# mryndzionek/composable-sdr

Measured on AMD Instinct MI355X. Metric: MS/s CF32 throughput, 256-ch PFB+FM pipeline, higher is better.
Workload: dtype f32; 1 GPU; cfg3: 256-ch firpfbch(m=7,As=80)+dcBlocker+freqdem(kf=0.3) on synthetic CF32, AGC off (-a 0), 262144 frames/step (512 MiB in, 256 MiB out), HBM-resident; channels=256, demod=fm, mix=False, route=fused-256|k_tile256<FM>, preheat_steps=12154, collective=none, rccl_ranks=1

## Files before the change

### composable_sdr_amd/csrc/fused_common.h

```cpp
#pragma once
#include "fused.h"
#include "run_split.h"

#include <cmath>
#include <cstdlib>
#include <vector>

namespace csdr {
namespace {

constexpr int M256 = 256;
constexpr int P = 14;
constexpr int NB = 16;
constexpr int FS_X = 272;
constexpr int FS_Z = 289;
constexpr int RS_Z = 18;
constexpr int RS_Y = 17;
constexpr int LDS_F2 = 16 * FS_Z;
constexpr int E_OFF = 4096;
constexpr int LOOKBACK = 10;
constexpr unsigned SPIN_LIMIT = 1u << 24;

typedef unsigned long long u64;
typedef float v2f __attribute__((ext_vector_type(2)));
// ... 310 lines not shown
{
    float2 s = T[tid & 15];
    float2 t;
    t = dpp2<0x111>(s); s = cfma(t, A.b256[1], s);
    t = dpp2<0x112>(s); s = cfma(t, A.b256[2], s);
    t = dpp2<0x114>(s); s = cfma(t, A.b256[4], s);
    t = dpp2<0x118>(s); s = cfma(t, A.b256[8], s);
    const int f = (tid >> 4) & 15;
    const int srcl = (tid & 48) | ((f - 1) & 15);
    float2 r = make_float2(__shfl(s.x, srcl), __shfl(s.y, srcl));
    return f ? r : make_float2(0.f, 0.f);
}


constexpr int WU = 6;


struct RunArgs {
    TileArgs t;
    RunSplit split;
    PhaseK pk;
    uint32_t nruns;
    float l2beta;
    uint32_t prio_div;
    uint32_t trace_light;
    const float4 *prev_tail;
    uint32_t indep;
    uint32_t pair_align;
    uint32_t wu_batch6;
    uint32_t wu, wu_rot;
    uint32_t tile_step;
    uint32_t nowu;
    float2 *cpre, *side;
};
constexpr int DCFIX_F = 113;

__device__ __forceinline__ float2 wg_sum(float2 v, float2 *red, int tid)
{
#pragma unroll
    for (int d = 32; d >= 1; d >>= 1) { v.x += __shfl_xor(v.x, d); v.y += __shfl_xor(v.y, d); }
    if ((tid & 63) == 0) red[tid >> 6] = v;
    __syncthreads();
    const float2 r = cadd(cadd(red[0], red[1]), cadd(red[2], red[3]));
    __syncthreads();
    return r;
}

__device__ __forceinline__ void row_scan4(float &x0, float &x1, float &x2, float &x3, float &s0, float &s1, float &s2, float &s3,
                                          float b1, float b2, float b4, float b8, float na)
{
    asm volatile(
        "v_mov_b32_e32 %4, %0\n\t"
        "v_mov_b32_e32 %5, %1\n\t"
        "v_mov_b32_e32 %6, %2\n\t"
        "v_mov_b32_e32 %7, %3\n\t"
        "v_fmac_f32_dpp %4, %4, %8 row_shr:1 row_mask:0xf bank_mask:0xf\n\t"
        "v_fmac_f32_dpp %5, %5, %8 row_shr:1 row_mask:0xf bank_mask:0xf\n\t"
        "v_fmac_f32_dpp %6, %6, %8 row_shr:1 row_mask:0xf bank_mask:0xf\n\t"
        "v_fmac_f32_dpp %7, %7, %8 row_shr:1 row_mask:0xf bank_mask:0xf\n\t"
        "v_fmac_f32_dpp %4, %4, %9 row_shr:2 row_mask:0xf bank_mask:0xf\n\t"
        "v_fmac_f32_dpp %5, %5, %9 row_shr:2 row_mask:0xf bank_mask:0xf\n\t"
        "v_fmac_f32_dpp %6, %6, %9 row_shr:2 row_mask:0xf bank_mask:0xf\n\t"
        "v_fmac_f32_dpp %7, %7, %9 row_shr:2 row_mask:0xf bank_mask:0xf\n\t"
        "v_fmac_f32_dpp %4, %4, %10 row_shr:4 row_mask:0xf bank_mask:0xf\n\t"
        "v_fmac_f32_dpp %5, %5, %10 row_shr:4 row_mask:0xf bank_mask:0xf\n\t"
        "v_fmac_f32_dpp %6, %6, %10 row_shr:4 row_mask:0xf bank_mask:0xf\n\t"
        "v_fmac_f32_dpp %7, %7, %10 row_shr:4 row_mask:0xf bank_mask:0xf\n\t"
        "v_fmac_f32_dpp %4, %4, %11 row_shr:8 row_mask:0xf bank_mask:0xf\n\t"
// ... 62 lines not shown
```

### composable_sdr_amd/csrc/fused_v2_common.h

```cpp
#pragma once
#include "fused_common.h"

namespace csdr {
namespace {

typedef float v4f __attribute__((ext_vector_type(4)));
#ifndef V2_DMA_AUX
#define V2_DMA_AUX ""
#endif
#ifndef V2_DMA_AUX_STREAM
#define V2_DMA_AUX_STREAM V2_DMA_AUX
#endif

__device__ __forceinline__ void bar()
{
    asm volatile("s_waitcnt lgkmcnt(0)\n\ts_barrier" ::: "memory");
}
__device__ __forceinline__ float opaque_v(float x) { asm volatile("" : "+v"(x)); return x; }

__device__ __forceinline__ unsigned dma_offset(int tid)
{
    const int wave = tid >> 6, lane = tid & 63;
    const int slot = 64 * wave + lane, q = slot >> 3, i = (slot & 7) ^ ((q >> 1) & 7);
    return (unsigned)(8 * q + i) * 16u;
// ... 97 lines not shown
#pragma unroll
    for (int i = 5; i >= 0; i--) {
        pA = __builtin_elementwise_fma(pA, zA, (v2f){k.c[i], k.c[i]});
        pB = __builtin_elementwise_fma(pB, zB, (v2f){k.c[i], k.c[i]});
    }
    const v2f tA = pA * sA, tB = pB * sB;
    const v2f hpv = {k.hp, k.hp}, piv = {k.pi, k.pi};
    const v2f thA = hpv - tA, thB = hpv - tB;
    const v2f uA = {sel_abs_gt(q[0].y, q[0].x, thA.x, tA.x), sel_abs_gt(q[1].y, q[1].x, thA.y, tA.y)};
    const v2f uB = {sel_abs_gt(q[2].y, q[2].x, thB.x, tB.x), sel_abs_gt(q[3].y, q[3].x, thB.y, tB.y)};
    const v2f wA = piv - uA, wB = piv - uB;
    m[0] = copysignf(sel_neg(q[0].x, wA.x, uA.x), q[0].y);
    m[1] = copysignf(sel_neg(q[1].x, wA.y, uA.y), q[1].y);
    m[2] = copysignf(sel_neg(q[2].x, wB.x, uB.x), q[2].y);
    m[3] = copysignf(sel_neg(q[3].x, wB.y, uB.y), q[3].y);
}

template <int CTRL> __device__ __forceinline__ float dpp_keep(float old, float v)
{
    return __int_as_float(__builtin_amdgcn_update_dpp(__float_as_int(old), __float_as_int(v), CTRL, 0xf, 0xf, false));
}

}
template <size_t OFF> __device__ __forceinline__ unsigned kernarg_u32_s()
{
    unsigned v = 0;
#if defined(__HIP_DEVICE_COMPILE__)
    typedef __attribute__((address_space(4))) const char *kptr;
    kptr ka = (kptr)__builtin_amdgcn_kernarg_segment_ptr();
    asm volatile("s_load_dword %0, %1, %2\n\ts_waitcnt lgkmcnt(0)" : "=s"(v) : "s"(ka), "n"(OFF) : "memory");
#endif
    return v;
}
template <size_t OFF> __device__ __forceinline__ float2 *kernarg_ptr_s()
{
    float2 *p = nullptr;
#if defined(__HIP_DEVICE_COMPILE__)
    typedef __attribute__((address_space(4))) const char *kptr;
    kptr ka = (kptr)__builtin_amdgcn_kernarg_segment_ptr();
    unsigned long long v;
    asm volatile("s_load_dwordx2 %0, %1, %2\n\ts_waitcnt lgkmcnt(0)" : "=s"(v) : "s"(ka), "n"(OFF) : "memory");
    p = reinterpret_cast<float2 *>(v);
#endif
    return p;
}

}
```

### composable_sdr_amd/csrc/kernels_fused.hip

```cpp
#include "fused_common.h"
#include <cstring>

namespace csdr {

namespace {

#define STAMP(i) do { if (A.trace && tid == 0) A.trace[(size_t)b * 16 + (i)] = __builtin_amdgcn_s_memtime(); } while (0)

template <bool FM>
__global__ __launch_bounds__(256) void k_tile256(TileArgs A)
{
    __shared__ __attribute__((aligned(16))) float2 R[LDS_F2];
    __shared__ float2 tw_s[M256];
    __shared__ float2 Tt[2][16];
    __shared__ float2 carry_s[2];
    __shared__ unsigned tile_s;

    const int tid = threadIdx.x;
    if (tid == 0) tile_s = atomicAdd(A.ticket, 1u);
    tw_s[tid] = A.tw[tid];
    __syncthreads();
    const unsigned b = tile_s;
    if (b >= A.nb) return;
    STAMP(0);
// ... 232 lines not shown
            for (int f = 0; f < NB; f++) if (f < nvalid) o[f] = v[f];
        }
    }
    STAMP(11);
}


}


__global__ __launch_bounds__(256) void k_save_tail(const float4 *__restrict__ src, float4 *__restrict__ dst)
{
    const unsigned i = blockIdx.x * 256u + threadIdx.x;
    dst[i] = src[i];
}

__global__ __launch_bounds__(64) void k_shard_gather(const float *__restrict__ src, float *__restrict__ dst, uint32_t c0, uint32_t G, uint32_t rem,
                                                     uint32_t nf, uint32_t t0, uint32_t w)
{
    const uint32_t m = blockIdx.x;
    for (uint32_t i = threadIdx.x; i < rem * w; i += 64) dst[((size_t)m * nf + t0) * w + i] = src[(size_t)(c0 + G * m) * rem * w + i];
}

struct FusedPlan : ChainPlan {
    using ChainPlan::ChainPlan;
    std::string kernel;
    uint32_t max_nb = 0, epoch = 0;
    float *d_taps = nullptr;
    float2 *d_tw = nullptr, *d_wpre = nullptr;
    float2 *d_yhist[2] = {nullptr, nullptr}, *d_vend[2] = {nullptr, nullptr}, *d_rp[2] = {nullptr, nullptr};
    unsigned *d_ticket = nullptr, *d_yflag = nullptr, *d_status = nullptr;
    u64 *d_agg = nullptr, *d_ylast = nullptr;
    float2 *d_cpre = nullptr, *d_side = nullptr, *d_rt = nullptr;
    bool nowu = false;
    u64 *d_trace = nullptr;
    uint32_t run_min_tiles = 1024;
    float slot_weight[8] = {1.f, 1.f, 1.f, 1.f, 1.f, 1.f, 1.f, 1.f};
    uint32_t slot_pairs[8] = {0, 0, 0, 0, 0, 0, 0, 0};
    bool have_pairs = false;
    uint32_t resident_wgs_v2 = 512;
    bool use_v3 = false;
    float *d_shard_tail = nullptr;
    float4 *d_tail[3] = {nullptr, nullptr, nullptr};
    int tail_w = 0;
    bool tail_valid = false, save_tails = false;
    TileArgs proto;

    int init();
    const char *name() const override { return kernel.c_str(); }
    bool tile_major_ok(uint32_t nf) const override;
    void keep_tail() override { save_tails = cfg.G == 1; }
    bool can_overlap(uint32_t nf) const override;
    bool tail_recorded() const override { return save_tails && tail_valid; }
    int status(unsigned *st) override;
    int trace(unsigned long long *out, uint32_t ntiles) override;
    int reset_state(hipStream_t s) override;
    int run(const FusedCall &call, void *out, hipStream_t s, KernelTimer *timer) override;
    bool v2_call(uint32_t nf) const { return cfg.G == 1 && cfg.c0 == 0 && cfg.C == cfg.M && nf / NB >= run_min_tiles; }
};

int ChainPlan::process(const FusedCall &call, hipStream_t s, KernelTimer *timer)
{
    if (!call.nf) return 0;
    if ((call.tile_major && !tile_major_ok(call.nf)) || (call.indep && !can_overlap(call.nf))) {
        set_error("fused: internal: tile-major output or an independent launch requested from a call that cannot run as one");
        return -1;
    }
// ... 60 lines not shown
    kernel = cfg.fm ? "k_tile256<FM>" : "k_tile256<CF32>";
    max_nb = (cfg.max_nf + NB - 1) / NB;
    if ((r = mem.alloc(&d_taps, sizeof(float) * cfg.M * cfg.p))) return r;
    if ((r = mem.alloc(&d_tw, sizeof(float2) * cfg.M))) return r;
    if ((r = mem.alloc(&d_wpre, sizeof(float2) * 2 * cfg.M))) return r;
    for (int i = 0; i < 2; i++) {
        if ((r = mem.alloc(&d_yhist[i], sizeof(float2) * 13 * cfg.M))) return r;
        if ((r = mem.alloc(&d_vend[i], sizeof(float2)))) return r;
        if ((r = mem.alloc(&d_rp[i], sizeof(float2) * (cfg.G > 1 ? cfg.M : cfg.C)))) return r;
    }
    if (cfg.G > 1 && (r = mem.alloc(&d_shard_tail, sizeof(float2) * cfg.M * NB))) return r;
    for (int i = 0; i < 3; i++) {
        if ((r = mem.alloc(&d_tail[i], sizeof(float4) * 2048 * (WU + 1)))) return r;
        CSDR_HIP(hipMemset(d_tail[i], 0, sizeof(float4) * 2048 * (WU + 1)));
    }
    tail_valid = true;
    if ((r = mem.alloc(&d_ticket, sizeof(unsigned)))) return r;
    if ((r = mem.alloc(&d_status, sizeof(unsigned)))) return r;
    if ((r = mem.alloc(&d_yflag, sizeof(unsigned) * max_nb))) return r;
    if ((r = mem.alloc(&d_agg, sizeof(u64) * 2 * max_nb))) return r;
    if ((r = mem.alloc(&d_ylast, sizeof(u64) * (size_t)cfg.M * max_nb))) return r;
    if (const char *e = diag_env("CSDR_RUN_MIN_TILES")) run_min_tiles = (uint32_t)atol(e);
    if (cfg.mix && (r = mem.alloc(&d_premix, (size_t)cfg.C * cfg.max_nf * (cfg.fm ? 4 : 8)))) return r;
    if (diag_env("CSDR_TRACE")) {
        if ((r = mem.alloc(&d_trace, sizeof(u64) * 16 * max_nb))) return r;
        CSDR_HIP(hipMemset(d_trace, 0, sizeof(u64) * 16 * max_nb));
    }
    nowu = cfg.G == 1 && cfg.c0 == 0 && cfg.C == cfg.M && cfg.dc_block && dc_window_ok(cfg.dc, (DCFIX_F - 1) * 256.0) &&
           !(diag_env("CSDR_NOWU") && atoi(diag_env("CSDR_NOWU")) == 0);
    if (nowu) {
        if ((r = mem.alloc(&d_cpre, sizeof(float2) * 2050))) return r;
        if ((r = mem.alloc(&d_side, sizeof(float2) * 2048 * 4 * DCFIX_F))) return r;
        if ((r = mem.alloc(&d_rt, sizeof(float2) * 2 * DCFIX_F * 4))) return r;
        CSDR_HIP(hipMemset(d_cpre, 0, sizeof(float2) * 2050));
    }
    CSDR_HIP(hipMemcpy(d_taps, cfg.taps, sizeof(float) * cfg.M * cfg.p, hipMemcpyHostToDevice));
    std::vector<float2> tw(cfg.M);
    for (uint32_t k1 = 0; k1 < 16; k1++)
        for (uint32_t b1 = 0; b1 < 16; b1++) {
            const double a = -2.0 * 3.14159265358979323846 * (double)(b1 * k1) / (double)cfg.M;
            tw[16 * k1 + b1] = make_float2((float)std::cos(a), (float)std::sin(a));
        }
    const std::vector<float2> wpre = premix_table();
    CSDR_HIP(hipMemcpy(d_tw, tw.data(), sizeof(float2) * cfg.M, hipMemcpyHostToDevice));
    CSDR_HIP(hipMemcpy(d_wpre, wpre.data(), sizeof(float2) * 2 * cfg.M, hipMemcpyHostToDevice));
    if (nowu) {
        std::vector<float2> rt((size_t)2 * DCFIX_F * 4);
        dc_state_response(cfg, wpre.data(), 15u, (uint32_t)DCFIX_F, 126u, rt.data());
        CSDR_HIP(hipMemcpy(d_rt, rt.data(), sizeof(float2) * rt.size(), hipMemcpyHostToDevice));
    }
    CSDR_HIP(hipMemset(d_status, 0, sizeof(unsigned)));
    CSDR_HIP(hipMemset(d_yflag, 0, sizeof(unsigned) * max_nb));
    CSDR_HIP(hipMemset(d_agg, 0, sizeof(u64) * 2 * max_nb));

    TileArgs &A = proto;
    A = TileArgs{};
    A.taps = d_taps; A.tw = d_tw; A.wpre = d_wpre;
    A.ticket = d_ticket; A.agg = d_agg; A.ylast = d_ylast; A.yflag = d_yflag; A.status = d_status;
    A.c0 = cfg.c0; A.C = cfg.C; A.fm_ref = cfg.fm_ref; A.trace = d_trace;
    const double beta = cfg.dc_block ? (double)cfg.dc.beta : 0.0;
    A.alpha = cfg.dc_block ? (float)(1.0 - beta) : 0.0f;
    A.beta = (float)beta;
    for (int k = 0; k < LOOKBACK + 2; k++) A.wtile[k] = (float)std::pow(beta, 4096.0 * k);
    for (int k = 0; k < 16; k++) A.b16[k] = (float)std::pow(beta, 16.0 * k);
    for (int k = 0; k < 17; k++) A.b256[k] = (float)std::pow(beta, 256.0 * k);
    for (int k = 0; k < 16; k++) A.bj[k] = (float)std::pow(beta, (double)k);
    if (const char *e = diag_env("CSDR_CUS")) { if (atoi(e) > 0 && (uint32_t)atoi(e) < cus) cus = (uint32_t)atoi(e); }
    resident_wgs_v2 = (uint32_t)(cus * run256_v2_blocks_per_cu(cfg.fm, cfg.G));
    if (const char *e = diag_env("CSDR_RESIDENT_WGS")) resident_wgs_v2 = (uint32_t)atol(e);
#ifdef CSDR_WITH_RUN256_V3
    if (const char *e = diag_env("CSDR_RUN_V3")) use_v3 = atoi(e) != 0;
#endif
    if (const char *e = diag_env("CSDR_RUN_WEIGHTS")) {
        int k = 0;
        for (const char *q = e; *q && k < 8; k++) { slot_weight[k] = (float)atof(q); q = strchr(q, ','); if (!q) break; q++; }
    }
    if (const char *e = diag_env("CSDR_RUN_PAIRS")) {
        int k = 0;
        for (const char *q = e; *q && k < 8; k++) { slot_pairs[k] = (uint32_t)atol(q); q = strchr(q, ','); if (!q) break; q++; }
        have_pairs = true;
    }
    return 0;
}

int FusedPlan::reset_state(hipStream_t s)
{
    for (int i = 0; i < 2; i++) {
        CSDR_HIP(hipMemsetAsync(d_yhist[i], 0, sizeof(float2) * 13 * cfg.M, s));
        CSDR_HIP(hipMemsetAsync(d_vend[i], 0, sizeof(float2), s));
        CSDR_HIP(hipMemsetAsync(d_rp[i], 0, sizeof(float2) * (cfg.G > 1 ? cfg.M : cfg.C), s));
    }
    CSDR_HIP(hipMemsetAsync(d_tail[0], 0, sizeof(float4) * 2048 * (WU + 1), s));
    tail_w = 0; tail_valid = true;
    return 0;
}

bool FusedPlan::tile_major_ok(uint32_t nf) const
{
    if (cfg.fm || cfg.mix || nf % NB || !nf) return false;
    if (cfg.G > 1) return (uint64_t)cfg.C * nf * 8u < (1ull << 32);
    return cfg.c0 == 0 && cfg.C == cfg.M && nf / NB >= run_min_tiles;
}

bool FusedPlan::can_overlap(uint32_t nf) const
{
    return save_tails && tail_valid && v2_call(nf) && nf % NB == 0 && !cfg.mix;
}

int FusedPlan::run(const FusedCall &call, void *out, hipStream_t s, KernelTimer *timer)
{
    const FusedConfig &c = cfg;
    const uint32_t nf = call.nf;
    int r;
    TileArgs A = proto;
    A.x = call.d_in;
    A.out = out;
    A.yhist_in = d_yhist[cur]; A.yhist_out = d_yhist[cur ^ 1];
    A.vend_in = d_vend[cur];   A.vend_out = d_vend[cur ^ 1];
    A.rp_in = d_rp[cur];       A.rp_out = d_rp[cur ^ 1];
    A.out_stride = nf; A.out_t0 = 0;
    if (call.tile_major) A.out_stride = NB;
    A.parity0 = (uint32_t)(frames_done & 1);
    const uint32_t nb_full = nf / NB;
    const bool shard = c.G > 1;
    if (shard && (uint64_t)c.C * nf * (c.fm ? 4u : 8u) >= (1ull << 32)) { set_error("fused: interleaved shard output of %u frames exceeds 4 GiB", nf); return -1; }
// ... 1 lines not shown
    if ((nb_full >= run_min_tiles && whole_band) || shard) {
        const bool v2 = true;
        const bool v3 = !shard && use_v3;
        kernel = v3 ? (c.fm ? "k_run256v3<FM>" : "k_run256v3<CF32>") : (c.fm ? "k_run256v2<FM>" : "k_run256v2<CF32>");
        if (shard) kernel += "/G" + std::to_string(c.G);
        RunArgs RA{};
        A.nf = nb_full * NB; A.nb = nb_full;
        RA.t = A; RA.pk = phase_consts(c.fm_ref);
        uint32_t nruns = v3 ? cus : resident_wgs_v2;
        if (v3) { if (const char *e = diag_env("CSDR_V3_RUNS")) nruns = (uint32_t)atol(e); }
        if (nruns > A.nb / 8) nruns = A.nb / 8;
        if (nruns < 1) nruns = 1;
        RA.nruns = nruns;
        static const float v2_weight_cf[8] = {1.2f, 0.8f, 1.f, 1.f, 1.f, 1.f, 1.f, 1.f};
        static const float v2_weight_fm[8] = {1.24f, 0.76f, 1.f, 1.f, 1.f, 1.f, 1.f, 1.f};
        static const float v2_weight_fm3[8] = {1.6f, 1.f, 0.6f, 1.f, 1.f, 1.f, 1.f, 1.f};
        const float *v2_weight = c.fm ? ((cus && nruns == 3 * cus) ? v2_weight_fm3 : v2_weight_fm) : v2_weight_cf;
        static const float equal_weight[8] = {1.f, 1.f, 1.f, 1.f, 1.f, 1.f, 1.f, 1.f};
        static const bool pd_equal = diag_env("CSDR_PD_EQUAL") != nullptr;
        RA.split = make_split(A.nb, nruns, cus, (call.indep && pd_equal) ? equal_weight : ((v2 && !diag_env("CSDR_RUN_WEIGHTS")) ? v2_weight : slot_weight),
                              have_pairs ? slot_pairs : nullptr);
        { const char *e = diag_env("CSDR_PRIO_ROT"); RA.prio_div = e ? (atoi(e) ? cus : 0u) : (v2 ? 0u : cus); }
        { const char *e = diag_env("CSDR_TRACE"); RA.trace_light = (e && atoi(e) == 2) ? 1u : 0u; }
        { const char *e = diag_env("CSDR_WU"); RA.wu = e ? (uint32_t)atoi(e) : (uint32_t)WU; }
        { const char *e = diag_env("CSDR_WU_ROT"); RA.wu_rot = e ? (uint32_t)atoi(e) : 0u; }
        RA.pair_align = (v2 && (c.fm || diag_env("CSDR_PAIR_ALIGN_CF"))) ? 1u : 0u;
        { const char *e = diag_env("CSDR_WU_BATCH6"); RA.wu_batch6 = e ? (uint32_t)atoi(e) : 1u; }
        RA.l2beta = c.dc_block ? (float)std::log2((double)c.dc.beta) : -1000.0f;
        RA.tile_step = call.tile_major ? c.C * 128u : (uint32_t)NB * (c.fm ? 4u : 8u);
        const bool whole = nf == nb_full * NB;
        RA.indep = call.indep ? 1u : 0u;
        RA.nowu = (nowu && !shard && !v3 && !RA.indep && nruns >= 2 && nruns <= 2048) ? 1u : 0u;
        RA.cpre = d_cpre; RA.side = d_side;
        RA.prev_tail = d_tail[tail_w];
        if (save_tails && !shard && v2 && whole && nb_full >= WU + 1) {
            const int nxt = (tail_w + 1) % 3;
            static const bool nocopy = diag_env("CSDR_PD_NOCOPY") != nullptr;
            if (!nocopy) hipLaunchKernelGGL(k_save_tail, dim3(2048 * (WU + 1) / 256), dim3(256), 0, s,
                                            reinterpret_cast<const float4 *>(call.d_in + (size_t)(nb_full - (WU + 1)) * 4096), d_tail[nxt]);
            if (call.ev_tail) CSDR_HIP(hipEventRecord(call.ev_tail, s));
            tail_w = nxt; tail_valid = true;
        } else tail_valid = false;
        if (timer && (r = timer->begin(s))) return r;
        if (nb_full == 0) {  }
#ifdef CSDR_WITH_RUN256_V3
        else if (v3) { if ((r = run256_v3_launch(&RA, c.fm, nruns, s))) return r; }
#endif
        else if ((r = run256_v2_launch(&RA, c.fm, c.G, nruns, s))) return r;
        if (RA.nowu && nb_full && (r = run256_dcfix_launch(&RA, c.fm, nruns, d_rt, s))) return r;
        if (timer && (r = timer->end(s))) return r;
        const uint32_t rem = nf - nb_full * NB;
        if (rem) {
            if (nb_full) cur ^= 1;
            TileArgs T = proto;
            T.x = call.d_in + (size_t)nb_full * NB * c.M; T.out = A.out;
            if (shard) { T.c0 = 0; T.C = c.M; T.out = d_shard_tail; }
            T.yhist_in = d_yhist[cur]; T.yhist_out = d_yhist[cur ^ 1];
            T.vend_in = d_vend[cur];   T.vend_out = d_vend[cur ^ 1];
            T.rp_in = d_rp[cur];       T.rp_out = d_rp[cur ^ 1];
            if (++epoch == 0) epoch = 1;
            T.epoch = epoch; T.nf = rem; T.nb = 1; T.out_stride = nf; T.out_t0 = nb_full * NB;
            if (shard) { T.out_stride = rem; T.out_t0 = 0; }
            T.parity0 = (uint32_t)((frames_done + nb_full * NB) & 1);
            CSDR_HIP(hipMemsetAsync(d_ticket, 0, sizeof(unsigned), s));
            if (c.fm) hipLaunchKernelGGL(k_tile256<true>, dim3(1), dim3(256), 0, s, T);
            else hipLaunchKernelGGL(k_tile256<false>, dim3(1), dim3(256), 0, s, T);
            if (shard) hipLaunchKernelGGL(k_shard_gather, dim3(c.C), dim3(64), 0, s, (const float *)d_shard_tail, (float *)A.out, c.c0, c.G, rem,
                                          nf, nb_full * NB, c.fm ? 1u : 2u);
        }
    } else {
        kernel = c.fm ? "k_tile256<FM>" : "k_tile256<CF32>";
        tail_valid = false;
        if (++epoch == 0) epoch = 1;
        A.epoch = epoch; A.nf = nf; A.nb = (nf + NB - 1) / NB;
        CSDR_HIP(hipMemsetAsync(d_ticket, 0, sizeof(unsigned), s));
        if (timer && (r = timer->begin(s))) return r;
        if (c.fm) hipLaunchKernelGGL(k_tile256<true>, dim3(A.nb), dim3(256), 0, s, A);
        else hipLaunchKernelGGL(k_tile256<false>, dim3(A.nb), dim3(256), 0, s, A);
        if (timer && (r = timer->end(s))) return r;
    }
    CSDR_HIP(hipGetLastError());
    return 0;
// ... 20 lines not shown
```

### composable_sdr_amd/csrc/kernels_fused_v2.hip

```cpp
#ifndef V2_FM_PACKED
#define V2_FM_PACKED 1
#endif
#ifndef V2_ABLATE
#define V2_ABLATE 0
#endif

#ifndef V2_COLSCAN
#define V2_COLSCAN 0
#endif
#ifndef V2_PAIR
#define V2_PAIR 1
#endif
#ifndef V2_STORE_AUX
#define V2_STORE_AUX ""
#endif
#ifndef V2_PAIR_CF
#define V2_PAIR_CF 0
#endif
#ifndef V2_BAR_E
#define V2_BAR_E 0
#endif
#ifndef V2_PAD
#define V2_PAD 1
#endif
#ifndef V2_ONE_WGS
#define V2_ONE_WGS 3
#endif
#ifndef V2_ONE_BURST
#define V2_ONE_BURST 1
#endif
#ifndef V2_SNOP
#define V2_SNOP ""
#endif

#include "fused_v2_common.h"
#include <cstddef>
#include <type_traits>

namespace csdr {
namespace {

constexpr unsigned V2_FSB = 2048u + (V2_PAD ? 128u : 0u);
constexpr int V2_FS2 = (int)V2_FSB / 8;
constexpr int V2_BUF = 16 * V2_FS2;
constexpr int V2_STASH = 2 * V2_BUF;
constexpr int V2_AUX2 = 256 + 32 + 256 + (V2_COLSCAN ? 512 : 0);
constexpr int V2_F2 = V2_STASH + V2_AUX2;
constexpr int V2_F2_ONE = V2_BUF + V2_AUX2 + P * M256 / 2;
#define V2_ZSW(f) (V2_PAD ? (((f) >> 1) & 7) : ((f) & 7))
#ifndef V2_RSWN
#define V2_RSWN V2_PAD
#endif
#define V2_RSW(a) (V2_RSWN ? ((a) & 7) : (((a) >> 1) & 7))

struct V2Args {
    RunArgs r;
};

template <bool FM, int G>
__global__ __launch_bounds__(256, (FM && G == 1) ? V2_ONE_WGS : 2) void k_run256v2(V2Args VA)
{
    static_assert(G == 1 || G == 2 || G == 4 || G == 8, "interleaved shards: G = 2, 4, 8");
    constexpr int NK1 = 16 / G;
    constexpr bool ONE = FM && G == 1;
    const RunArgs &RA = VA.r;
    const TileArgs &A = RA.t;
    __shared__ __attribute__((aligned(16))) float2 L[(ONE && V2_ONE_WGS >= 3) ? V2_F2_ONE : V2_F2];
    float2 *R = L, *ST = L + (ONE ? V2_BUF : V2_STASH), *Tt = ST + 256, *red = Tt + 16;
    float2 *tw_s = red + 16;
    float2 *TRc = tw_s + 256, *Ec = TRc + 256;
    (void)TRc; (void)Ec;
    float *TP = reinterpret_cast<float *>(L + (ONE ? V2_BUF : V2_STASH) + V2_AUX2);
    float2 *H = ONE ? L : L + V2_BUF;
    float2 *HS = ONE ? reinterpret_cast<float2 *>(TP) : H;
    float2 *E = ST;
    const int tid = threadIdx.x, j = tid;
    const unsigned w = blockIdx.x;
    unsigned first, last;
    run_range(RA.split, w, first, last);
    if (RA.pair_align) {
        first &= ~1u;
        if (last != A.nb) last &= ~1u;
    }
    const float4 *x4 = reinterpret_cast<const float4 *>(A.x);
    const int col_off = 16 * (j >> 4) + 2 * (((j & 15) >> 1) ^ V2_RSW(j >> 4)) + (j & 1);
    const unsigned goff = V2_RSWN ? dma_offset_rsw(tid) : dma_offset(tid);
    const unsigned wave_u = (unsigned)__builtin_amdgcn_readfirstlane(tid >> 6);
    const unsigned lds_wave = (unsigned)(size_t)(__attribute__((address_space(3))) float2 *)R + V2_FSB * (wave_u >> 1) + 1024u * (wave_u & 1u);

#ifndef V2_TRACE
// ... 121 lines not shown
    const int st_i = XIDX(tid >> 4), st_j1 = ((tid & 15) - (int)(G > 1 ? A.c0 : 0u)) / G;
    const bool st_own = G == 1 || ((((tid & 15) - (int)A.c0) & (G - 1)) == 0 && (tid & 15) >= (int)A.c0);
    const int st_idx = G == 1 ? (tid & 15) * 16 + st_i : (st_own ? ((st_i / NK1) * NK1 + st_j1) * 16 + st_i : 0);
    if (st_own) ST[st_idx] = (FM && !cold) ? A.rp_in[tid] : make_float2(0.f, 0.f);
    __syncthreads();
    if (FM && cold) {
        w2 = cmul(w2, Wa);
        v2f acc = {0.f, 0.f};
#pragma unroll
        for (int n = P - 1; n >= 0; n--) {
            const float2 s2 = (n == P - 1) ? w2 : wa[NB - 1 - n];
            acc = __builtin_elementwise_fma((v2f){s2.x, s2.y}, (v2f){h[n], h[n]}, acc);
        }
        HS[j] = to_f2(acc);
        __syncthreads();
        v2f vv[16];
        if (tid < 16) {
#pragma unroll
            for (int a = 0; a < 16; a++) vv[a] = to_v(HS[16 * a + tid]);
            fft16_v(vv);
#pragma unroll
            for (int i = (G > 1 ? 0 : 1); i < 16; i++) vv[i] = cmul_v(vv[i], to_v(tw_s[16 * ((XIDX(i) + (G > 1 ? (int)A.c0 : 0)) & 15) + tid]));
#pragma unroll
            for (int i = 0; i < 16; i++) HS[256 + 16 * XIDX(i) + tid] = to_f2(vv[i]);
        }
        __syncthreads();
        if (tid < 16) {
#pragma unroll
            for (int b = 0; b < 16; b++) vv[b] = to_v(HS[256 + 16 * (G * (tid % NK1)) + b]);
            fft16_v(vv);
#pragma unroll
            for (int i = 0; i < 16; i++) ST[tid * 16 + i] = to_f2(vv[i]);
            if (G == 1 && RA.nowu) {
                if (tid >= 14) RA.side[((size_t)w * 4 + (tid - 14)) * DCFIX_F] = to_f2(vv[13]);
                else if (tid <= 1) RA.side[((size_t)w * 4 + 2 + tid) * DCFIX_F] = to_f2(vv[2]);
            }
        }
        __syncthreads();
    }

    if (ONE) {
#pragma unroll
        for (int n = 0; n < P; n++) TP[M256 * n + j] = h[n];
    }
    const v2f Wav = to_v(Wa), Wbv = to_v(Wb);
    const float na = opaque_v(-A.alpha), be = opaque_v(A.beta);
    const float kJ = -A.alpha * exp2f((float)j * RA.l2beta);
    const float b256 = A.b256[1];
    const FmK2 fk = {{opaque_v(9.999993443e-01f), opaque_v(-3.332985938e-01f), opaque_v(1.994656026e-01f), opaque_v(-1.390860826e-01f),
                      opaque_v(9.642146528e-02f), opaque_v(-5.591168255e-02f), opaque_v(2.186254039e-02f), opaque_v(-4.054457881e-03f)},
                     opaque_v(1e-37f), opaque_v(A.fm_ref), opaque_v(RA.pk.hp), opaque_v(RA.pk.pi)};
    const int q = tid, sw = V2_RSW(q & 15);
    const unsigned raw_a_ = (unsigned)q * 128u + (unsigned)(q >> 4) * (V2_FSB - 2048u) + ((unsigned)sw << 4);
    const int f1 = tid >> 4, b1 = tid & 15;
    const int k1 = tid >> 4, f2 = tid & 15;
    const unsigned x_a_ = (unsigned)f1 * V2_FSB + (unsigned)b1 * 8u;
    const unsigned zw_a = (unsigned)f1 * V2_FSB + (unsigned)((((b1 >> 1) ^ V2_ZSW(f1)) << 1) | (b1 & 1)) * 8u;
    const unsigned z_a_ = (unsigned)f2 * V2_FSB + (unsigned)k1 * 128u + ((unsigned)V2_ZSW(f2) << 4);
    const int j1 = k1 % NK1, hb = (G == 8) ? ((k1 >> 1) & 1) : 0;
    const unsigned z_a_g = (unsigned)f2 * V2_FSB + (unsigned)(G * j1) * 128u + ((unsigned)V2_ZSW(f2) << 4);
    const uint32_t voff = ((uint32_t)(G == 1 ? k1 : j1 + 16 * hb) * A.out_stride + A.out_t0 + (uint32_t)f2) * (FM ? 4u : 8u);
    const size_t row16 = (size_t)NK1 * A.out_stride * (FM ? 4u : 8u);
#if V2_TRACE
#define V2STAMP(i) do { if (A.trace && !RA.trace_light && tid == 0) A.trace[(size_t)b_ * 16 + (i)] = __builtin_amdgcn_s_memtime(); } while (0)
#else
#define V2STAMP(i) do { } while (0)
#endif

    float hold[16];
    v2f holdc[V2_PAIR_CF ? 16 : 1];
    auto tile = [&](float2 (&old)[NB], float2 (&nw)[NB], unsigned b_, const int par) {
        unsigned b = (unsigned)__builtin_amdgcn_readfirstlane((int)b_);
        asm volatile("" : "+s"(b));
        char *B = reinterpret_cast<char *>(L) + (ONE ? 0 : par) * (V2_BUF * 8);
        float2 *Bf = reinterpret_cast<float2 *>(B);
        if (RA.prio_div) {
            if (((b_ - first) + w / RA.prio_div) & 1u) __builtin_amdgcn_s_setprio(1); else __builtin_amdgcn_s_setprio(0);
        }
        int tid_t = tid;
        if (ONE) asm volatile("" : "+v"(tid_t));
        V2STAMP(0);
        if (G == 1 && b + 1 == last && tid == 0) {
            if (kernarg_u32_s<offsetof(V2Args, r.nowu)>()) kernarg_ptr_s<offsetof(V2Args, r.cpre)>()[w + 1] = c;
        }
        if (V2_TRACE && A.trace && !RA.trace_light && tid == 0) A.trace[(size_t)b_ * 16 + 15] = __builtin_amdgcn_s_memrealtime();
        bar();
        V2STAMP(1);
#ifdef V2_SELECTIVE_POLICY
        if (!(V2_ABLATE & 1) && b + 1 < last) {
            if (b + 1 + (WU + 1) < last) dma_tile<true, 2 * V2_FSB>(x4 + (size_t)(b + 1) * 2048, goff, lds_wave + (unsigned)(par ^ 1) * (V2_BUF * 8u));
            else dma_tile<false, 2 * V2_FSB>(x4 + (size_t)(b + 1) * 2048, goff, lds_wave + (unsigned)(par ^ 1) * (V2_BUF * 8u));
        }
#else
        if (!ONE && !(V2_ABLATE & 1) && b + 1 < last) dma_tile<false, 2 * V2_FSB>(x4 + (size_t)(b + 1) * 2048, goff, lds_wave + (unsigned)(par ^ 1) * (V2_BUF * 8u));
#endif
        auto next_pieces = [&](const int it) {
            if (ONE && !(V2_ABLATE & 1) && b + 1 < last) {
                dma_piece<2 * V2_FSB>(x4 + (size_t)(b + 1) * 2048, goff, lds_wave, it);
                dma_piece<2 * V2_FSB>(x4 + (size_t)(b + 1) * 2048, goff, lds_wave, it + 1);
            }
        };
#if V2_COLSCAN
#pragma unroll
        for (int f = 0; f < NB; f++) nw[f] = Bf[V2_FS2 * f + col_off];
        col_run_scan(nw, TRc, A, tid);
        V2STAMP(2);
        bar();
        col_run_carries(TRc, Ec, Tt, A, tid);
        bar();
        V2STAMP(3);
        {
            v2f V = to_v(c);
            const float kj = -A.alpha * A.bj[j & 15];
            const v2f kJv = {kJ, kJ}, bv = {b256, b256}, kjv = {kj, kj};
#pragma unroll
            for (int f = 0; f < NB; f++) {
// ... 166 lines not shown
                        for (int u = 0; u < NS; u += 2) *reinterpret_cast<v4f *>(stp + u) = (v4f){y[u].x, y[u].y, y[u + 1].x, y[u + 1].y};
                    }
                } else {
#pragma unroll
                    for (int u = 0; u < NS; u++) {
                        const char *rowp = obase + (size_t)XIDX(S0 + u) * row16;
                        asm volatile("s_nop 4\n\tglobal_store_dwordx2 %0, %1, %2\n\ts_nop 1" :: "v"(voff), "v"(y[u]), "s"(rowp) : "memory");
                    }
                }
            };
            if (G == 2) { if (wave_u < 2u) shard_tail(std::integral_constant<int, 0>{}); else shard_tail(std::integral_constant<int, 2>{}); }
            else switch (wave_u) {
                case 0: shard_tail(std::integral_constant<int, 0>{}); break;
                case 1: shard_tail(std::integral_constant<int, 1>{}); break;
                case 2: shard_tail(std::integral_constant<int, 2>{}); break;
                default: shard_tail(std::integral_constant<int, 3>{}); break;
            }
            V2STAMP(14);
            return;
        }
        const unsigned z_a = ONE ? (unsigned)(tid_t & 15) * V2_FSB + (unsigned)(tid_t >> 4) * 128u + ((unsigned)V2_ZSW(tid_t & 15) << 4) : z_a_;
#pragma unroll
        for (int i = 0; i < 8; i++) {
            const v4f v = *reinterpret_cast<const v4f *>(B + (z_a ^ (unsigned)(i << 4)));
            vv[2 * i] = (v2f){v.x, v.y}; vv[2 * i + 1] = (v2f){v.z, v.w};
        }
        if (ONE) {
            bar();
            next_pieces(0);
            if (V2_ONE_BURST) { next_pieces(2); next_pieces(4); next_pieces(6); }
        }
        if (!(V2_ABLATE & 16)) fft16_v(vv);
        V2STAMP(11);
        if (G == 1 && cold && b - first < 7u && kernarg_u32_s<offsetof(V2Args, r.nowu)>()) {
            const int k1s = ONE ? tid_t >> 4 : k1, f2s = ONE ? tid_t & 15 : f2;
            float2 *sd = kernarg_ptr_s<offsetof(V2Args, r.side)>() + ((size_t)w * 4) * DCFIX_F + 1 + 16 * (size_t)(b - first) + f2s;
            if (k1s >= 14) sd[(k1s - 14) * DCFIX_F] = to_f2(vv[13]);
            else if (k1s <= 1) sd[(2 + k1s) * DCFIX_F] = to_f2(vv[2]);
        }
        char *obase = reinterpret_cast<char *>(A.out) + (size_t)b * RA.tile_step;
        if (FM) {
            if (!ONE) asm volatile("s_waitcnt vmcnt(0)" ::: "memory");
#pragma unroll
            for (int i = 0; i < 16; i += 4) {
                float2 rp[4], rr[4];
#pragma unroll
                for (int u = 0; u < 4; u += 2) {
                    const v4f sp = *reinterpret_cast<const v4f *>(ST + k1 * 16 + i + u);
                    rp[u] = make_float2(dpp_keep<0x111>(sp.x, vv[i + u].x), dpp_keep<0x111>(sp.y, vv[i + u].y));
                    rp[u + 1] = make_float2(dpp_keep<0x111>(sp.z, vv[i + u + 1].x), dpp_keep<0x111>(sp.w, vv[i + u + 1].y));
                    rr[u] = to_f2(vv[i + u]); rr[u + 1] = to_f2(vv[i + u + 1]);
                }
                float mq_[4];
                float (&mq)[4] = (V2_PAIR && par == 0) ? *reinterpret_cast<float (*)[4]>(&hold[i]) : mq_;
                if (V2_ABLATE & 4) { mq[0] = rp[0].x + rr[0].y; mq[1] = rp[1].y + rr[1].x; mq[2] = rp[2].x + rr[2].y; mq[3] = rp[3].y + rr[3].x; }
                else if (V2_FM_PACKED) fm_quad(rp, rr, fk, mq);
                else {
                    const FmK k1s = {fk.tiny, fk.ref, fk.hp, fk.pi};
#pragma unroll
                    for (int u = 0; u < 4; u++) mq[u] = fm_sample(rp[u], rr[u], k1s);
                }
                if (!V2_ONE_BURST && i < 12) next_pieces(2 + i / 2);
                if (V2_PAIR && par == 0 && b + 1 < last) continue;
#pragma unroll
                for (int u = 0; u < 4; u++) {
                    const char *rowp = obase + (size_t)XIDX(i + u) * row16;
                    if (V2_ABLATE & 2) asm volatile("" :: "v"(mq[u]), "s"(rowp));
                    else {
                        if (V2_PAIR && par == 1) asm volatile(V2_SNOP "global_store_dword %0, %1, %2 offset:-64" V2_STORE_AUX :: "v"(voff), "v"(hold[i + u]), "s"(rowp) : "memory");
                        asm volatile(V2_SNOP "global_store_dword %0, %1, %2" V2_STORE_AUX :: "v"(voff), "v"(mq[u]), "s"(rowp) : "memory");
                    }
                }
            }
            if (f2 == 15) {
#pragma unroll
                for (int i = 0; i < 16; i += 2) *reinterpret_cast<v4f *>(ST + k1 * 16 + i) = (v4f){vv[i].x, vv[i].y, vv[i + 1].x, vv[i + 1].y};
            }
            if (ONE && b + 1 < last) {
                if ((V2_PAIR && par == 0) || (V2_ABLATE & 2)) asm volatile("s_waitcnt vmcnt(0)" ::: "memory");
                else asm volatile("s_waitcnt vmcnt(%0)" :: "n"((V2_ONE_BURST ? 4 : 2) * (V2_PAIR ? 8 : 4)) : "memory");
            }
            V2STAMP(12);
            V2STAMP(13);
        } else {
            V2STAMP(12);
            asm volatile("s_waitcnt vmcnt(0)" ::: "memory");
            V2STAMP(13);
            if (V2_PAIR_CF && par == 0 && b + 1 < last) {
#pragma unroll
                for (int i = 0; i < 16; i++) holdc[i] = vv[i];
            } else {
#pragma unroll
                for (int i = 0; i < 16; i++) {
                    const char *rowp = obase + (size_t)XIDX(i) * row16;
                    if (V2_ABLATE & 2) asm volatile("" :: "v"(vv[i]), "s"(rowp));
                    else {
                        if (V2_PAIR_CF && par == 1) asm volatile(V2_SNOP "global_store_dwordx2 %0, %1, %2 offset:-128" V2_STORE_AUX :: "v"(voff), "v"(holdc[i]), "s"(rowp) : "memory");
                        asm volatile(V2_SNOP "global_store_dwordx2 %0, %1, %2" V2_STORE_AUX :: "v"(voff), "v"(vv[i]), "s"(rowp) : "memory");
                    }
                }
            }
        }
        V2STAMP(14);
    };

    V2LSTAMP(2);
    asm volatile("s_waitcnt vmcnt(0)" ::: "memory");
    V2LSTAMP(3);
    for (unsigned b = first; b < last; b += 2) {
        tile(wa, wb, b, 0);
        if (b + 1 >= last) break;
        tile(wb, wa, b + 1, 1);
    }

    V2LSTAMP(4);
    bar();
    if (FM) {
        const float2 lastY = ST[st_idx];
        if (last == A.nb && st_own) A.rp_out[tid] = lastY;
    }
    if (last == A.nb && tid == 0) A.vend_out[0] = c;
}

}

template <bool FM>
__global__ __launch_bounds__(128) void k_run256_dcfix(V2Args VA, const float2 *__restrict__ Rt)
{
    const RunArgs &RA = VA.r;
    const TileArgs &A = RA.t;
    __shared__ float2 Ys[4][DCFIX_F + 1];
    const unsigned w = blockIdx.x + 1;
    unsigned first, last;
    run_range(RA.split, w, first, last);
    if (RA.pair_align) { first &= ~1u; if (last != A.nb) last &= ~1u; }
    if (first >= last || first <= 1) return;
    const int t = threadIdx.x;
    const float2 c = RA.cpre[w];
    const float2 *R = Rt + (size_t)(A.parity0 & 1u) * DCFIX_F * 4;
    float2 y[4];
    if (t < DCFIX_F) {
#pragma unroll
        for (int ch = 0; ch < 4; ch++) {
            const float2 r = R[t * 4 + ch], s0 = RA.side[((size_t)w * 4 + ch) * DCFIX_F + t];
            y[ch] = make_float2(fmaf(c.x, r.x, fmaf(-c.y, r.y, s0.x)), fmaf(c.x, r.y, fmaf(c.y, r.x, s0.y)));
            Ys[ch][t] = y[ch];
        }
    }
    __syncthreads();
    if (t < 1 || t >= DCFIX_F) return;
    const unsigned b = first + (unsigned)(t - 1) / 16u, f2 = (unsigned)(t - 1) & 15u;
    if (b >= last) return;
    char *obase = reinterpret_cast<char *>(A.out) + (size_t)b * RA.tile_step;
    const FmK fk = {1e-37f, A.fm_ref, RA.pk.hp, RA.pk.pi};
#pragma unroll
    for (int ch = 0; ch < 4; ch++) {
        const size_t off = ((size_t)(126 + ch) * A.out_stride + A.out_t0 + f2) * (FM ? 4u : 8u);
        if (FM) *reinterpret_cast<float *>(obase + off) = fm_sample(Ys[ch][t - 1], y[ch], fk);
        else *reinterpret_cast<float2 *>(obase + off) = y[ch];
    }
}

int run256_dcfix_launch(const void *run_args, bool fm, unsigned nruns, const float2 *Rt, hipStream_t s)
{
    if (nruns < 2) return 0;
    V2Args VA;
    VA.r = *static_cast<const RunArgs *>(run_args);
    if (fm) hipLaunchKernelGGL(k_run256_dcfix<true>, dim3(nruns - 1), dim3(128), 0, s, VA, Rt);
    else hipLaunchKernelGGL(k_run256_dcfix<false>, dim3(nruns - 1), dim3(128), 0, s, VA, Rt);
    return 0;
}

static V2Args make_v2(const void *run_args)
{
    V2Args VA;
    VA.r = *static_cast<const RunArgs *>(run_args);
    return VA;
}

int run256_v2_launch(const void *run_args, bool fm, unsigned G, unsigned nruns, hipStream_t s)
{
    const V2Args VA = make_v2(run_args);
#define V2_LAUNCH(F, GG) hipLaunchKernelGGL((k_run256v2<F, GG>), dim3(nruns), dim3(256), 0, s, VA)
    if (G == 1) { if (fm) V2_LAUNCH(true, 1); else V2_LAUNCH(false, 1); }
    else if (G == 2) { if (fm) V2_LAUNCH(true, 2); else V2_LAUNCH(false, 2); }
    else if (G == 4) { if (fm) V2_LAUNCH(true, 4); else V2_LAUNCH(false, 4); }
    else if (G == 8) { if (fm) V2_LAUNCH(true, 8); else V2_LAUNCH(false, 8); }
    else { set_error("k_run256v2: interleaved shards of stride %u are not built (2, 4, 8)", G); return -1; }
#undef V2_LAUNCH
    return 0;
}

int run256_v2_blocks_per_cu(bool fm, unsigned G)
{
    int occ = 0;
    if (G != 1) { if (fm) (void)hipOccupancyMaxActiveBlocksPerMultiprocessor(&occ, (k_run256v2<true, 2>), 256, 0);
                  else (void)hipOccupancyMaxActiveBlocksPerMultiprocessor(&occ, (k_run256v2<false, 2>), 256, 0); }
    else if (fm) (void)hipOccupancyMaxActiveBlocksPerMultiprocessor(&occ, (k_run256v2<true, 1>), 256, 0);
    else (void)hipOccupancyMaxActiveBlocksPerMultiprocessor(&occ, (k_run256v2<false, 1>), 256, 0);
    return occ < 1 ? 1 : occ;
}

// ... 2 lines not shown
```

Baseline: 311,400 MS/s.

## Fold DC-fix pass into main run kernel via ticket handoff between neighbouring runs

Adds an optional fold mode in which the last of each pair of adjacent workgroups, chosen with an atomic ticket, applies the DC-fix correction for its own run or its successor inside the main v2 kernel. This removes the separate dcfix kernel launch. Side and cpre values are now written and read with agent-scope atomics so another workgroup can see them. The fold path is off by default (dcfix_launch=true unless the env var clears it), so by default only the standalone dcfix kernel changes: it now uses 256 threads and the shared apply routine, and DCFIX_F grows from 113 to 129, so the fix window covers 8 tiles instead of 7.

```diff
diff --git a/composable_sdr_amd/csrc/fused_common.h b/composable_sdr_amd/csrc/fused_common.h
--- a/composable_sdr_amd/csrc/fused_common.h
+++ b/composable_sdr_amd/csrc/fused_common.h
@@ -366,8 +366,11 @@
     uint32_t tile_step;
     uint32_t nowu;
     float2 *cpre, *side;
+    uint32_t fold;
+    unsigned *ticket2;
+    const float2 *rt;
 };
-constexpr int DCFIX_F = 113;
+constexpr int DCFIX_F = 129;
 
 __device__ __forceinline__ float2 wg_sum(float2 v, float2 *red, int tid)
 {
diff --git a/composable_sdr_amd/csrc/fused_v2_common.h b/composable_sdr_amd/csrc/fused_v2_common.h
--- a/composable_sdr_amd/csrc/fused_v2_common.h
+++ b/composable_sdr_amd/csrc/fused_v2_common.h
@@ -153,6 +153,17 @@
 #endif
     return v;
 }
+__device__ __forceinline__ unsigned kernarg_u32_sd(unsigned off)
+{
+    unsigned v = 0;
+#if defined(__HIP_DEVICE_COMPILE__)
+    typedef __attribute__((address_space(4))) const char *kptr;
+    kptr ka = (kptr)__builtin_amdgcn_kernarg_segment_ptr();
+    off = (unsigned)__builtin_amdgcn_readfirstlane((int)off);
+    asm volatile("s_load_dword %0, %1, %2\n\ts_waitcnt lgkmcnt(0)" : "=s"(v) : "s"(ka), "s"(off) : "memory");
+#endif
+    return v;
+}
 template <size_t OFF> __device__ __forceinline__ float2 *kernarg_ptr_s()
 {
     float2 *p = nullptr;
diff --git a/composable_sdr_amd/csrc/kernels_fused.hip b/composable_sdr_amd/csrc/kernels_fused.hip
--- a/composable_sdr_amd/csrc/kernels_fused.hip
+++ b/composable_sdr_amd/csrc/kernels_fused.hip
@@ -288,7 +288,8 @@
     unsigned *d_ticket = nullptr, *d_yflag = nullptr, *d_status = nullptr;
     u64 *d_agg = nullptr, *d_ylast = nullptr;
     float2 *d_cpre = nullptr, *d_side = nullptr, *d_rt = nullptr;
-    bool nowu = false;
+    unsigned *d_ticket2 = nullptr;
+    bool nowu = false, dcfix_launch = true;
     u64 *d_trace = nullptr;
     uint32_t run_min_tiles = 1024;
     float slot_weight[8] = {1.f, 1.f, 1.f, 1.f, 1.f, 1.f, 1.f, 1.f};
@@ -415,7 +416,10 @@
         if ((r = mem.alloc(&d_cpre, sizeof(float2) * 2050))) return r;
         if ((r = mem.alloc(&d_side, sizeof(float2) * 2048 * 4 * DCFIX_F))) return r;
         if ((r = mem.alloc(&d_rt, sizeof(float2) * 2 * DCFIX_F * 4))) return r;
+        if ((r = mem.alloc(&d_ticket2, sizeof(unsigned) * 2050))) return r;
         CSDR_HIP(hipMemset(d_cpre, 0, sizeof(float2) * 2050));
+        CSDR_HIP(hipMemset(d_ticket2, 0, sizeof(unsigned) * 2050));
+        if (const char *e = diag_env("CSDR_DCFIX_LAUNCH")) dcfix_launch = atoi(e) != 0;
     }
     CSDR_HIP(hipMemcpy(d_taps, cfg.taps, sizeof(float) * cfg.M * cfg.p, hipMemcpyHostToDevice));
     std::vector<float2> tw(cfg.M);
@@ -474,6 +478,7 @@
         CSDR_HIP(hipMemsetAsync(d_rp[i], 0, sizeof(float2) * (cfg.G > 1 ? cfg.M : cfg.C), s));
     }
     CSDR_HIP(hipMemsetAsync(d_tail[0], 0, sizeof(float4) * 2048 * (WU + 1), s));
+    if (d_ticket2) CSDR_HIP(hipMemsetAsync(d_ticket2, 0, sizeof(unsigned) * 2050, s));
     tail_w = 0; tail_valid = true;
     return 0;
 }
@@ -541,6 +546,8 @@
         RA.indep = call.indep ? 1u : 0u;
         RA.nowu = (nowu && !shard && !v3 && !RA.indep && nruns >= 2 && nruns <= 2048) ? 1u : 0u;
         RA.cpre = d_cpre; RA.side = d_side;
+        RA.fold = (RA.nowu && c.fm && !dcfix_launch) ? 1u : 0u;
+        RA.ticket2 = d_ticket2; RA.rt = d_rt;
         RA.prev_tail = d_tail[tail_w];
         if (save_tails && !shard && v2 && whole && nb_full >= WU + 1) {
             const int nxt = (tail_w + 1) % 3;
@@ -556,7 +563,7 @@
         else if (v3) { if ((r = run256_v3_launch(&RA, c.fm, nruns, s))) return r; }
 #endif
         else if ((r = run256_v2_launch(&RA, c.fm, c.G, nruns, s))) return r;
-        if (RA.nowu && nb_full && (r = run256_dcfix_launch(&RA, c.fm, nruns, d_rt, s))) return r;
+        if (RA.nowu && !RA.fold && nb_full && (r = run256_dcfix_launch(&RA, c.fm, nruns, d_rt, s))) return r;
         if (timer && (r = timer->end(s))) return r;
         const uint32_t rem = nf - nb_full * NB;
         if (rem) {
diff --git a/composable_sdr_amd/csrc/kernels_fused_v2.hip b/composable_sdr_amd/csrc/kernels_fused_v2.hip
--- a/composable_sdr_amd/csrc/kernels_fused_v2.hip
+++ b/composable_sdr_amd/csrc/kernels_fused_v2.hip
@@ -56,6 +56,57 @@
 struct V2Args {
     RunArgs r;
 };
+
+typedef __attribute__((address_space(1))) unsigned long long gu64;
+typedef __attribute__((address_space(1))) unsigned gu32;
+__device__ __forceinline__ void st_sc1(float2 *p, float2 v)
+{
+    __hip_atomic_store((gu64 *)p, ((unsigned long long)__float_as_uint(v.y) << 32) | __float_as_uint(v.x), __ATOMIC_RELAXED, __HIP_MEMORY_SCOPE_AGENT);
+}
+__device__ __forceinline__ float2 ld_sc1(const float2 *p)
+{
+    const unsigned long long v = __hip_atomic_load((const gu64 *)p, __ATOMIC_RELAXED, __HIP_MEMORY_SCOPE_AGENT);
+    return make_float2(__uint_as_float((unsigned)v), __uint_as_float((unsigned)(v >> 32)));
+}
+
+struct DcfixK {
+    const float2 *cpre, *side, *rt;
+    void *out;
+    uint32_t out_stride, out_t0, parity0, tile_step;
+    float fm_ref, hp, pi;
+};
+template <bool FM>
+__device__ __forceinline__ void dcfix_apply(const DcfixK &K, unsigned w, unsigned first, unsigned last, float2 (*Ys)[DCFIX_F + 1], int t)
+{
+    const float2 c = ld_sc1(K.cpre + w);
+    const float2 *R = K.rt + (size_t)(K.parity0 & 1u) * DCFIX_F * 4;
+    const int cp = 2 * (t >> 7), fr = t & 127;
+    float2 y[2];
+#pragma unroll
+    for (int u = 0; u < 2; u++) {
+        const float2 *sd = K.side + ((size_t)w * 4 + (cp + u)) * DCFIX_F;
+        const float2 r = R[(fr + 1) * 4 + cp + u], s0 = ld_sc1(sd + fr + 1);
+        y[u] = make_float2(fmaf(c.x, r.x, fmaf(-c.y, r.y, s0.x)), fmaf(c.x, r.y, fmaf(c.y, r.x, s0.y)));
+        Ys[cp + u][fr + 1] = y[u];
+        if (fr == 0) {
+            const float2 rm = R[cp + u], sm = ld_sc1(sd);
+            Ys[cp + u][0] = make_float2(fmaf(c.x, rm.x, fmaf(-c.y, rm.y, sm.x)), fmaf(c.x, rm.y, fmaf(c.y, rm.x, sm.y)));
+        }
+    }
+    __syncthreads();
+    const unsigned b = first + (unsigned)fr / 16u, f2 = (unsigned)fr & 15u;
+    if (b < last) {
+        char *obase = reinterpret_cast<char *>(K.out) + (size_t)b * K.tile_step;
+        const FmK fk = {1e-37f, K.fm_ref, K.hp, K.pi};
+#pragma unroll
+        for (int u = 0; u < 2; u++) {
+            const size_t off = ((size_t)(126 + cp + u) * K.out_stride + K.out_t0 + f2) * (FM ? 4u : 8u);
+            if (FM) *reinterpret_cast<float *>(obase + off) = fm_sample(Ys[cp + u][fr], y[u], fk);
+            else *reinterpret_cast<float2 *>(obase + off) = y[u];
+        }
+    }
+    __syncthreads();
+}
 
 template <bool FM, int G>
 __global__ __launch_bounds__(256, (FM && G == 1) ? V2_ONE_WGS : 2) void k_run256v2(V2Args VA)
@@ -243,8 +294,8 @@
 #pragma unroll
             for (int i = 0; i < 16; i++) ST[tid * 16 + i] = to_f2(vv[i]);
             if (G == 1 && RA.nowu) {
-                if (tid >= 14) RA.side[((size_t)w * 4 + (tid - 14)) * DCFIX_F] = to_f2(vv[13]);
-                else if (tid <= 1) RA.side[((size_t)w * 4 + 2 + tid) * DCFIX_F] = to_f2(vv[2]);
+                if (tid >= 14) st_sc1(RA.side + ((size_t)w * 4 + (tid - 14)) * DCFIX_F, to_f2(vv[13]));
+                else if (tid <= 1) st_sc1(RA.side + ((size_t)w * 4 + 2 + tid) * DCFIX_F, to_f2(vv[2]));
             }
         }
         __syncthreads();
@@ -292,7 +343,7 @@
         if (ONE) asm volatile("" : "+v"(tid_t));
         V2STAMP(0);
         if (G == 1 && b + 1 == last && tid == 0) {
-            if (kernarg_u32_s<offsetof(V2Args, r.nowu)>()) kernarg_ptr_s<offsetof(V2Args, r.cpre)>()[w + 1] = c;
+            if (kernarg_u32_s<offsetof(V2Args, r.nowu)>()) st_sc1(kernarg_ptr_s<offsetof(V2Args, r.cpre)>() + (w + 1), c);
         }
         if (V2_TRACE && A.trace && !RA.trace_light && tid == 0) A.trace[(size_t)b_ * 16 + 15] = __builtin_amdgcn_s_memrealtime();
         bar();
@@ -525,11 +576,13 @@
         }
         if (!(V2_ABLATE & 16)) fft16_v(vv);
         V2STAMP(11);
-        if (G == 1 && cold && b - first < 7u && kernarg_u32_s<offsetof(V2Args, r.nowu)>()) {
+        const bool fix8 = G == 1 && cold && b - first < 8u && kernarg_u32_s<offsetof(V2Args, r.nowu)>();
+        const bool skip = ONE && fix8 && first > 1u && kernarg_u32_s<offsetof(V2Args, r.fold)>();
+        if (fix8) {
             const int k1s = ONE ? tid_t >> 4 : k1, f2s = ONE ? tid_t & 15 : f2;
             float2 *sd = kernarg_ptr_s<offsetof(V2Args, r.side)>() + ((size_t)w * 4) * DCFIX_F + 1 + 16 * (size_t)(b - first) + f2s;
-            if (k1s >= 14) sd[(k1s - 14) * DCFIX_F] = to_f2(vv[13]);
-            else if (k1s <= 1) sd[(2 + k1s) * DCFIX_F] = to_f2(vv[2]);
+            if (k1s >= 14) st_sc1(sd + (k1s - 14) * DCFIX_F, to_f2(vv[13]));
+            else if (k1s <= 1) st_sc1(sd + (2 + k1s) * DCFIX_F, to_f2(vv[2]));
         }
         char *obase = reinterpret_cast<char *>(A.out) + (size_t)b * RA.tile_step;
         if (FM) {
@@ -558,6 +611,8 @@
 #pragma unroll
                 for (int u = 0; u < 4; u++) {
                     const char *rowp = obase + (size_t)XIDX(i + u) * row16;
+                    if (ONE && i + u == 13 && skip && tid_t >= 224) continue;
+                    if (ONE && i + u == 2 && skip && tid_t < 32) continue;
                     if (V2_ABLATE & 2) asm volatile("" :: "v"(mq[u]), "s"(rowp));
                     else {
                         if (V2_PAIR && par == 1) asm volatile(V2_SNOP "global_store_dword %0, %1, %2 offset:-64" V2_STORE_AUX :: "v"(voff), "v"(hold[i + u]), "s"(rowp) : "memory");
@@ -613,12 +668,56 @@
         if (last == A.nb && st_own) A.rp_out[tid] = lastY;
     }
     if (last == A.nb && tid == 0) A.vend_out[0] = c;
+    if constexpr (ONE) {
+        if (kernarg_u32_s<offsetof(V2Args, r.fold)>()) {
+            unsigned nfirst = 0, nlast = 0;
+            const unsigned w1 = w + 1u;
+            const bool succ = w1 < kernarg_u32_s<offsetof(V2Args, r.nruns)>();
+            if (succ) {
+                const unsigned rps = kernarg_u32_s<offsetof(V2Args, r.split.rps)>(), shift = kernarg_u32_s<offsetof(V2Args, r.split.shift)>();
+                const unsigned sl = w1 / rps, i = w1 - sl * rps;
+                const unsigned base = kernarg_u32_sd((unsigned)offsetof(V2Args, r.split.base) + 4u * sl);
+                const unsigned tiles = kernarg_u32_sd((unsigned)offsetof(V2Args, r.split.tiles) + 4u * sl), n = tiles >> shift;
+                nfirst = base + ((uint32_t)((unsigned long long)i * n / rps) << shift);
+                nlast = base + (i + 1 == rps ? tiles : ((uint32_t)((unsigned long long)(i + 1) * n / rps) << shift));
+                if (kernarg_u32_s<offsetof(V2Args, r.pair_align)>()) {
+                    nfirst &= ~1u;
+                    if (nlast != kernarg_u32_s<offsetof(V2Args, r.t.nb)>()) nlast &= ~1u;
+                }
+            }
+            unsigned wq = w, fq = first, lq = last;
+            asm volatile("" : "+s"(wq), "+s"(fq), "+s"(lq));
+            const bool own = wq > 0u && fq > 1u && fq < lq, nxt = succ && nfirst > 1u && nfirst < nlast;
+            unsigned *arrived = reinterpret_cast<unsigned *>(red);
+            asm volatile("s_waitcnt vmcnt(0)" ::: "memory");
+            __syncthreads();
+            if (tid == 0) {
+                gu32 *tk = (gu32 *)kernarg_ptr_s<offsetof(V2Args, r.ticket2)>();
+                arrived[0] = own ? __hip_atomic_fetch_add(tk + w, 1u, __ATOMIC_RELAXED, __HIP_MEMORY_SCOPE_AGENT) : 0u;
+                arrived[1] = nxt ? __hip_atomic_fetch_add(tk + w1, 1u, __ATOMIC_RELAXED, __HIP_MEMORY_SCOPE_AGENT) : 0u;
+            }
+            __syncthreads();
+            const bool do_own = own && (arrived[0] & 1u), do_nxt = nxt && (arrived[1] & 1u);
+            if (do_own || do_nxt) {
+                DcfixK K;
+                K.cpre = kernarg_ptr_s<offsetof(V2Args, r.cpre)>(); K.side = kernarg_ptr_s<offsetof(V2Args, r.side)>();
+                K.rt = kernarg_ptr_s<offsetof(V2Args, r.rt)>(); K.out = kernarg_ptr_s<offsetof(V2Args, r.t.out)>();
+                K.out_stride = kernarg_u32_s<offsetof(V2Args, r.t.out_stride)>(); K.out_t0 = kernarg_u32_s<offsetof(V2Args, r.t.out_t0)>();
+                K.parity0 = kernarg_u32_s<offsetof(V2Args, r.t.parity0)>(); K.tile_step = kernarg_u32_s<offsetof(V2Args, r.tile_step)>();
+                K.fm_ref = __uint_as_float(kernarg_u32_s<offsetof(V2Args, r.t.fm_ref)>());
+                K.hp = __uint_as_float(kernarg_u32_s<offsetof(V2Args, r.pk.hp)>()); K.pi = __uint_as_float(kernarg_u32_s<offsetof(V2Args, r.pk.pi)>());
+                float2 (*Ys)[DCFIX_F + 1] = reinterpret_cast<float2 (*)[DCFIX_F + 1]>(L);
+                if (do_own) dcfix_apply<true>(K, w, first, last, Ys, tid);
+                if (do_nxt) dcfix_apply<true>(K, w1, nfirst, nlast, Ys, tid);
+            }
+        }
+    }
 }
 
 }
 
 template <bool FM>
-__global__ __launch_bounds__(128) void k_run256_dcfix(V2Args VA, const float2 *__restrict__ Rt)
+__global__ __launch_bounds__(256) void k_run256_dcfix(V2Args VA, const float2 *__restrict__ Rt)
 {
     const RunArgs &RA = VA.r;
     const TileArgs &A = RA.t;
@@ -628,30 +727,8 @@
     run_range(RA.split, w, first, last);
     if (RA.pair_align) { first &= ~1u; if (last != A.nb) last &= ~1u; }
     if (first >= last || first <= 1) return;
-    const int t = threadIdx.x;
-    const float2 c = RA.cpre[w];
-    const float2 *R = Rt + (size_t)(A.parity0 & 1u) * DCFIX_F * 4;
-    float2 y[4];
-    if (t < DCFIX_F) {
-#pragma unroll
-        for (int ch = 0; ch < 4; ch++) {
-            const float2 r = R[t * 4 + ch], s0 = RA.side[((size_t)w * 4 + ch) * DCFIX_F + t];
-            y[ch] = make_float2(fmaf(c.x, r.x, fmaf(-c.y, r.y, s0.x)), fmaf(c.x, r.y, fmaf(c.y, r.x, s0.y)));
-            Ys[ch][t] = y[ch];
-        }
-    }
-    __syncthreads();
-    if (t < 1 || t >= DCFIX_F) return;
-    const unsigned b = first + (unsigned)(t - 1) / 16u, f2 = (unsigned)(t - 1) & 15u;
-    if (b >= last) return;
-    char *obase = reinterpret_cast<char *>(A.out) + (size_t)b * RA.tile_step;
-    const FmK fk = {1e-37f, A.fm_ref, RA.pk.hp, RA.pk.pi};
-#pragma unroll
-    for (int ch = 0; ch < 4; ch++) {
-        const size_t off = ((size_t)(126 + ch) * A.out_stride + A.out_t0 + f2) * (FM ? 4u : 8u);
-        if (FM) *reinterpret_cast<float *>(obase + off) = fm_sample(Ys[ch][t - 1], y[ch], fk);
-        else *reinterpret_cast<float2 *>(obase + off) = y[ch];
-    }
+    const DcfixK K = {RA.cpre, RA.side, Rt, A.out, A.out_stride, A.out_t0, A.parity0, RA.tile_step, A.fm_ref, RA.pk.hp, RA.pk.pi};
+    dcfix_apply<FM>(K, w, first, last, Ys, (int)threadIdx.x);
 }
 
 int run256_dcfix_launch(const void *run_args, bool fm, unsigned nruns, const float2 *Rt, hipStream_t s)
@@ -659,8 +736,8 @@
     if (nruns < 2) return 0;
     V2Args VA;
     VA.r = *static_cast<const RunArgs *>(run_args);
-    if (fm) hipLaunchKernelGGL(k_run256_dcfix<true>, dim3(nruns - 1), dim3(128), 0, s, VA, Rt);
-    else hipLaunchKernelGGL(k_run256_dcfix<false>, dim3(nruns - 1), dim3(128), 0, s, VA, Rt);
+    if (fm) hipLaunchKernelGGL(k_run256_dcfix<true>, dim3(nruns - 1), dim3(256), 0, s, VA, Rt);
+    else hipLaunchKernelGGL(k_run256_dcfix<false>, dim3(nruns - 1), dim3(256), 0, s, VA, Rt);
     return 0;
 }
 
```

After: 309,500 MS/s. No clear change (-0.6%).
